# MPF-Optimization-Laboratory/ConicIP.jl

Hardware: NVIDIA B200
Metric: kkt_factor_plus_solves_per_sec (higher is better)
Workload: dtype f64

## Files before the change

conicip.jl_b200/csrc/engine.cu:

```cuda
#include <climits>
#include <stdarg.h>
#include <stdlib.h>
#include <string.h>

#include <math.h>

#include <algorithm>
#include <vector>

#include "engine.h"
#include "nccl_dl.h"

namespace cip {

static thread_local char g_err[1024] = "";
std::atomic<long long> g_launches{0};

int sm_count() {
  static std::atomic<int> cache[64];
  int dev = 0;
  if (cudaGetDevice(&dev) != cudaSuccess || dev < 0 || dev >= 64) return 148;
  int v = cache[dev].load(std::memory_order_relaxed);
  if (v == 0) {
    if (cudaDeviceGetAttribute(&v, cudaDevAttrMultiProcessorCount, dev) != cudaSuccess || v <= 0) v = 148;
// ... 559 lines not shown
    if (cone_type[i] == CIP_CONE_Q) { qlist.push_back(i); maxq = std::max(maxq, cone_dim[i]); }
    else if (cone_type[i] == CIP_CONE_S) {
      const int k = (int)((sqrt(1.0 + 8.0 * cone_dim[i]) - 1.0) / 2.0 + 0.5);
      if (k * (k + 1) / 2 != cone_dim[i]) {
        set_error("S cone %d: dimension %d is not k(k+1)/2", i, cone_dim[i]);
        return -1;
      }
      if (k > sdp_max_order()) {
        set_error("S cone %d: order %d exceeds the supported maximum %d", i, k, sdp_max_order());
        return -2;
      }
      slist.push_back(i);
      h->h_sord.push_back(k);
      h->h_roff.push_back((int)h->r_total);
      h->r_total += (size_t)k * k;
      maxs = std::max(maxs, k);
    }
    else if (cone_type[i] != CIP_CONE_R) {
      set_error("unknown cone type %d", cone_type[i]);
      return -1;
    }
  }
  if (h->h_off[ncones] != m) {
    set_error("cone dimensions sum to %d but A has %d rows", h->h_off[ncones], m);
    return -1;
  }
  CIP_TRY(dev_alloc(h, &h->d_type, ncones));
  CIP_TRY(dev_alloc(h, &h->d_off, ncones + 1));
  CIP_TRY(dev_alloc(h, &h->d_rowcone, m));
  CIP_TRY(dev_alloc(h, &h->d_qlist, qlist.size()));
  CIP_TRY(dev_alloc(h, &h->d_slist, slist.size()));
  CIP_TRY(dev_alloc(h, &h->d_sord, slist.size()));
  CIP_TRY(dev_alloc(h, &h->d_roff, slist.size()));
  h->h_slist = slist;
  if (ncones) CIP_CUDA(cudaMemcpy(h->d_type, h->h_type.data(), sizeof(int) * ncones, cudaMemcpyHostToDevice));
  CIP_CUDA(cudaMemcpy(h->d_off, h->h_off.data(), sizeof(int) * (ncones + 1), cudaMemcpyHostToDevice));
  if (m) CIP_CUDA(cudaMemcpy(h->d_rowcone, rowcone.data(), sizeof(int) * m, cudaMemcpyHostToDevice));
  if (!qlist.empty())
    CIP_CUDA(cudaMemcpy(h->d_qlist, qlist.data(), sizeof(int) * qlist.size(), cudaMemcpyHostToDevice));
  if (!slist.empty()) {
    CIP_CUDA(cudaMemcpy(h->d_slist, slist.data(), sizeof(int) * slist.size(), cudaMemcpyHostToDevice));
    CIP_CUDA(cudaMemcpy(h->d_sord, h->h_sord.data(), sizeof(int) * slist.size(), cudaMemcpyHostToDevice));
    CIP_CUDA(cudaMemcpy(h->d_roff, h->h_roff.data(), sizeof(int) * slist.size(), cudaMemcpyHostToDevice));
  }
  h->cd.m = m; h->cd.ncones = ncones; h->cd.type = h->d_type; h->cd.off = h->d_off;
  h->cd.row_cone = h->d_rowcone; h->cd.qlist = h->d_qlist; h->cd.nq = (int)qlist.size();
  h->cd.slist = h->d_slist; h->cd.ns = (int)slist.size(); h->cd.max_q_dim = maxq; h->cd.max_s_ord = maxs;
  h->cd.sord = h->d_sord; h->cd.roff = h->d_roff;
  h->cd.sws = nullptr; h->cd.sws_stride = sdp_workspace_doubles(maxs);
  if (h->cd.sws_stride > 0) {
    const long long ctas = (long long)slist.size() * std::max(1, sdp_panel_chunks(maxs, n));
    CIP_TRY(dev_alloc(h, &h->d_sws, (size_t)(ctas * h->cd.sws_stride)));
    h->cd.sws = h->d_sws;
  }
  h->cd.nr_rows = 0;
  for (int i = 0; i < ncones; ++i)
    if (cone_type[i] == CIP_CONE_R) h->cd.nr_rows += h->h_off[i + 1] - h->h_off[i];
  for (Scaling* S : {&h->F, &h->Fi}) {
    CIP_TRY(dev_alloc(h, &S->kind, ncones));
    CIP_TRY(dev_alloc(h, &S->a, h->m_pad + 4));
    CIP_TRY(dev_alloc(h, &S->b, h->m_pad + 4));
    CIP_TRY(dev_alloc(h, &S->D, ncones));
  }
  CIP_TRY(dev_alloc(h, &h->F.R, h->r_total));
  CIP_TRY(dev_alloc(h, &h->F.Ri, h->r_total));
  h->Fi.R = h->F.R;
  h->Fi.Ri = h->F.Ri;

  const size_t nn = (size_t)h->n_pad * h->n_pad;
  const size_t mn = (size_t)h->m_pad * h->n_pad;
  if (!(h->rs.on && As)) CIP_TRY(dev_alloc(h, &h->At4, mn));
  {
    double rho = h->opt.aug_rho;
    if (rho < 0) rho = (p > 0) ? 1.0 : 0.0;
    h->aug_rho = (p > 0) ? rho : 0.0;
    h->aug_rows = (h->aug_rho > 0) ? round_up(p, 32) : 0;
  }
  if (!h->rs.on) CIP_TRY(engine_decide_fold(h, slist.empty() && qlist.empty() && h->aug_rows == 0 && m > 0, mn, &h->fold));
  if (!h->rs.on && !h->fold) CIP_TRY(fast_syrk_plan(h, slist.empty() && qlist.empty() && h->aug_rows == 0 && m > 0));
  if (h->fast.on) CIP_TRY(dev_alloc(h, &h->Atil4, fast_syrk_atil_doubles(h)));
  else if (!h->fold && !h->rs.on) CIP_TRY(dev_alloc(h, &h->Atil4, (size_t)(h->m_pad + h->aug_rows) * h->n_pad));
  const bool split = h->rs.sp.on;
  if (!split || (!Qs && h->opt.q_kind == 0)) CIP_TRY(dev_alloc(h, &h->Qq4, nn));
  if (!split) CIP_TRY(dev_alloc(h, &h->H4, nn));
  CIP_TRY(dev_alloc(h, &h->gemm_ws, (size_t)GEMM_WS_DOUBLES));
  if (!split) CIP_TRY(dev_alloc(h, &h->Winv, (size_t)h->n_pad * TILE));
  CIP_TRY(dev_alloc(h, &h->info, 4));
  cudaStream_t s = h->stream;

  if (Qs && split) {
    CIP_TRY(split_classify_csc_Q(h, Qs));
  } else if (Qs) {
    CIP_TRY(upload_csc(h, h->Qq4, h->n_pad, Qs, 0));
  } else if (h->opt.q_kind == 0) {
    if (!Q) { set_error("Q is null"); return -1; }
    if (kernel_readable(Q, h->device)) {
      CIP_TRY(pack_rows_q4(h->Qq4, h->n_pad, Q, ldq, n, n, h->n_pad, h->n_pad, s));
    } else {
      const int chunk = std::max(4, std::min(n, (int)((256u << 20) / ((size_t)n * 8)) / 4 * 4));
      double* stg = nullptr;
      CIP_CUDA(cudaMalloc(&stg, (size_t)n * chunk * 8));
      for (int c0 = 0; c0 < n; c0 += chunk) {
        const int nc = std::min(chunk, n - c0);
        CIP_CUDA(cudaMemcpy2DAsync(stg, (size_t)n * 8, Q + (size_t)c0 * ldq, (size_t)ldq * 8, (size_t)n * 8, nc,
                                   cudaMemcpyDefault, s));
        CIP_TRY(pack_rows_q4(h->Qq4 + (size_t)(c0 / 4) * h->n_pad * 4, h->n_pad, stg, n, n, nc, h->n_pad,
                             round_up(nc, 4), s));
        CIP_CUDA(cudaStreamSynchronize(s));
      }
      cudaFree(stg);
    }
  } else if (h->opt.q_kind == 1) {
    if (!Q) { set_error("Q (diagonal) is null"); return -1; }
    if (split) {
      CIP_TRY(split_diag_Q(h, Q));
    } else {
      double* dq = nullptr;
      CIP_CUDA(cudaMalloc(&dq, sizeof(double) * n));
      CIP_CUDA(cudaMemcpyAsync(dq, Q, sizeof(double) * n, cudaMemcpyDefault, s));
      CIP_TRY(set_diag_vec_q4(h->Qq4, h->n_pad, n, dq, s));
      CIP_CUDA(cudaStreamSynchronize(s));
      cudaFree(dq);
    }
  }
  if (h->Qq4) CIP_TRY(add_diag_q4(h->Qq4, h->n_pad, n, h->n_pad, 1.0, 1, s));

  if (m > 0) {
    if (!A && !As) { set_error("A is null"); return -1; }
    if (As && h->rs.on) {
      CIP_TRY(structure_build_csc(h, As));
    } else if (As) {
      CIP_TRY(upload_csc(h, h->At4, h->n_pad, As, 1));
    } else if (kernel_readable(A, h->device)) {
      CIP_TRY(pack_trans_q4(h->At4, h->n_pad, 0, A, lda, m, h->m_pad, n, s));
    } else {
      const int chunk = std::max(1, std::min(n, (int)((512u << 20) / ((size_t)m * 8))));
      double* stg = nullptr;
      CIP_CUDA(cudaMalloc(&stg, (size_t)m * chunk * 8));
      for (int c0 = 0; c0 < n; c0 += chunk) {
        const int nc = std::min(chunk, n - c0);
        CIP_CUDA(cudaMemcpy2DAsync(stg, (size_t)m * 8, A + (size_t)c0 * lda, (size_t)lda * 8, (size_t)m * 8, nc,
                                   cudaMemcpyDefault, s));
        CIP_TRY(pack_trans_q4(h->At4, h->n_pad, c0, stg, m, m, h->m_pad, nc, s));
        CIP_CUDA(cudaStreamSynchronize(s));
      }
      cudaFree(stg);
    }
    if (h->rs.on && !As) CIP_TRY(structure_build_dense(h));
  }
  if (h->rs.on) {
  } else if (h->fold) {
    CIP_TRY(make_q4_tensor_map(&h->mapAt.map, h->At4, h->n_pad, h->m_pad / 4));
  } else if (h->fast.on) {
    CIP_TRY(make_q4_tensor_map(&h->mapAtil.map, h->Atil4, h->n_pad, (long long)h->fast.K2));
    CIP_TRY(fast_syrk_setup(h));
  } else if (h->m_pad + h->aug_rows > 0) {
    CIP_TRY(make_q4_tensor_map(&h->mapAtil.map, h->Atil4, h->n_pad, (h->m_pad + h->aug_rows) / 4));
  }
  if (!split) CIP_TRY(chol_make_plan(&h->cholH, h->H4, h->n_pad, h->Winv, h->info));

  if (p > 0) {
    if (!G && !Gs) { set_error("G is null"); return -1; }
    const size_t pn = (size_t)h->p_pad * h->n_pad;
    CIP_TRY(dev_alloc(h, &h->G4, pn));
    if (!split) CIP_TRY(dev_alloc(h, &h->Z4, pn));
    CIP_TRY(dev_alloc(h, &h->S4, (size_t)h->p_pad * h->p_pad));
    CIP_TRY(dev_alloc(h, &h->Sbase4, (size_t)h->p_pad * h->p_pad));
    CIP_TRY(dev_alloc(h, &h->WinvS, (size_t)h->p_pad * TILE));
    if (Gs) {
      CIP_TRY(upload_csc(h, h->G4, h->p_pad, Gs, 0));
    } else {
      double* stg = nullptr;
      const double* gsrc = G;
      int gld = ldg;
      if (!kernel_readable(G, h->device)) {
        CIP_CUDA(cudaMalloc(&stg, (size_t)p * n * 8));
        CIP_CUDA(cudaMemcpy2DAsync(stg, (size_t)p * 8, G, (size_t)ldg * 8, (size_t)p * 8, n, cudaMemcpyDefault, s));
        gsrc = stg;
        gld = p;
      }
      CIP_TRY(pack_rows_q4(h->G4, h->p_pad, gsrc, gld, p, n, h->p_pad, h->n_pad, s));
      CIP_CUDA(cudaStreamSynchronize(s));
      if (stg) cudaFree(stg);
    }
    if (h->aug_rows > 0 && !h->rs.on)
      CIP_TRY(transpose_scale_q4(h->Atil4, h->n_pad, h->m_pad, h->G4, h->p_pad, p, n, sqrt(h->aug_rho), s));
    CIP_TRY(add_diag_q4(h->Sbase4, h->p_pad, p, h->p_pad, 1.0, 1, s));
    if (h->opt.reg_eps_G != 0.0) CIP_TRY(add_diag_q4(h->Sbase4, h->p_pad, 0, p, h->opt.reg_eps_G, 1, s));
    if (!split) CIP_TRY(make_q4_tensor_map(&h->mapZ.map, h->Z4, h->p_pad, h->n_pad / 4));
    CIP_TRY(chol_make_plan(&h->cholS, h->S4, h->p_pad, h->WinvS, h->info + 1));
  }
  if (h->rs.on) CIP_TRY(structure_finish(h));

  for (auto& v : h->nv) CIP_TRY(dev_alloc(h, &v, h->n_pad + 4));
  for (auto& v : h->mv) CIP_TRY(dev_alloc(h, &v, h->m_pad + 4));
  for (auto& v : h->pv) CIP_TRY(dev_alloc(h, &v, h->p_pad + 4));
  h->partial_cap = 4 * sm_count() * 8 * 128 + 64 * std::max(n, std::max(p, 1));
  CIP_TRY(dev_alloc(h, &h->partial, h->partial_cap));
  CIP_TRY(dev_alloc(h, &h->scalar, 8));
  CIP_CUDA(cudaStreamSynchronize(s));
  h->st.n = n; h->st.m = m; h->st.p = p; h->st.n_pad = h->n_pad; h->st.m_pad = h->m_pad; h->st.p_pad = h->p_pad;
  return 0;
}

}

namespace cip {
int engine_create_single(cip_handle* out, int n, int m, int p, const double* Q, int ldq, const double* A, int lda,
                         const double* G, int ldg, const cip_csc* Qs, const cip_csc* As, const cip_csc* Gs,
                         int ncones, const int* cone_type, const int* cone_dim, const cip_options* opts) {
  return create_impl(out, n, m, p, Q, ldq, A, lda, G, ldg, Qs, As, Gs, ncones, cone_type, cone_dim, opts,
                     true);
}
}

namespace {
bool wants_multi(const cip_options* opts) {
  return opts && (size_t)opts->struct_size >= offsetof(cip_options, ngpus) + sizeof(int) && opts->ngpus > 1;
}
bool reject_sharded_structure(const cip_options* opts) {
  if (opts && (size_t)opts->struct_size >= offsetof(cip_options, row_structure) + sizeof(int) &&
      opts->row_structure != 0) {
    set_error("row_structure is supported on single-device handles only (ngpus = %d)", opts->ngpus);
    return true;
  }
  return false;
}
}

extern "C" {

int cip_create(cip_handle* out, int n, int m, int p, const double* Q, int ldq, const double* A, int lda,
               const double* G, int ldg, int ncones, const int* cone_type, const int* cone_dim,
               const cip_options* opts) {
  if (wants_multi(opts)) {
    if (!out || n <= 0 || m < 0 || p < 0 || ncones < 0 || (ncones > 0 && (!cone_type || !cone_dim))) {
      set_error("cip_create: bad dimensions n=%d m=%d p=%d ncones=%d", n, m, p, ncones);
      return -1;
    }
    if (reject_sharded_structure(opts)) return -1;
    return multi_create(out, n, m, p, Q, ldq, A, lda, G, ldg, nullptr, nullptr, nullptr, ncones, cone_type,
                        cone_dim, opts);
  }
  return create_impl(out, n, m, p, Q, ldq, A, lda, G, ldg, nullptr, nullptr, nullptr, ncones, cone_type, cone_dim,
                     opts);
}

int cip_create_csc(cip_handle* out, int n, const cip_csc* Q, const cip_csc* A, const cip_csc* G, int ncones,
                   const int* cone_type, const int* cone_dim, const cip_options* opts) {
  if (!A || A->ncols != n || (Q && (Q->nrows != n || Q->ncols != n)) || (G && G->nrows > 0 && G->ncols != n)) {
    set_error("cip_create_csc: inconsistent matrix shapes");
    return -1;
  }
  cip_options o{};
  o.dist_chol = -1;
  o.aug_rho = -1.0;
  if (opts) memcpy(&o, opts, std::min<size_t>(sizeof(o), (size_t)opts->struct_size));
  else o.device = -1;
  o.struct_size = sizeof(o);
  o.q_kind = 2;
  const int p = G ? G->nrows : 0;
  if (wants_multi(&o)) {
    if (!out || n <= 0 || ncones < 0 || (ncones > 0 && (!cone_type || !cone_dim))) {
      set_error("cip_create_csc: bad arguments");
      return -1;
    }
    if (reject_sharded_structure(&o)) return -1;
    return multi_create(out, n, A->nrows, p, nullptr, 0, nullptr, 0, nullptr, 0, Q, A, (p > 0) ? G : nullptr, ncones,
                        cone_type, cone_dim, &o);
  }
  return create_impl(out, n, A->nrows, p, nullptr, 0, nullptr, 0, nullptr, 0, Q, A, (p > 0) ? G : nullptr, ncones,
                     cone_type, cone_dim, &o);
}

int cip_destroy(cip_handle h) {
  if (!h) return 0;
  if (h->multi) return multi_destroy(h);
  cudaSetDevice(h->device);
  if (h->own_stream) cudaStreamSynchronize(h->stream);
  if (h->comm) {
    const NcclApi* api = nccl_api();
    if (api) api->CommDestroy(h->comm);
  }
  void* ptrs[] = {h->At4, h->Atil4, h->Qq4, h->H4, h->Winv, h->G4, h->Z4, h->S4, h->Sbase4, h->WinvS, h->info,
                  h->d_type, h->d_off, h->d_rowcone, h->d_qlist, h->d_slist, h->F.kind, h->F.a, h->F.b, h->F.D,
                  h->Fi.kind, h->Fi.a, h->Fi.b, h->Fi.D, h->partial, h->scalar, h->F.R, h->F.Ri, h->d_sord, h->d_roff, h->gemm_ws};
  for (void* p : ptrs) if (p) cudaFree(p);
  for (void* p : h->owned) cudaFree(p);
  for (auto v : h->nv) if (v) cudaFree(v);
  for (auto v : h->mv) if (v) cudaFree(v);
  for (auto v : h->pv) if (v) cudaFree(v);
  for (auto v : h->nv2) if (v) cudaFree(v);
  for (auto v : h->mv2) if (v) cudaFree(v);
  for (auto v : h->pv2) if (v) cudaFree(v);
  chol_free_plan(&h->cholH);
  chol_free_plan(&h->cholS);
  chol_free_plan(&h->rs.sp.chol);
  if (h->Hp) cudaFree(h->Hp);
  if (h->d_sws) cudaFree(h->d_sws);
  if (h->cs) cudaStreamDestroy(h->cs);
  if (h->s2) cudaStreamDestroy(h->s2);
  for (auto e : h->evc) if (e) cudaEventDestroy(e);
  for (auto e : h->ev) if (e) cudaEventDestroy(e);
  if (h->own_stream) cudaStreamDestroy(h->own_stream);
  cudaGetLastError();
  delete h;
  return 0;
// ... 513 lines not shown
```

conicip.jl_b200/csrc/engine.h:

```cpp
#pragma once
#include <vector>

#include "../../include/conicip_b200.h"
#include "kernels.cuh"

constexpr int NV = 8;
constexpr int MV = 10;
constexpr int PV = 6;

namespace cip {
struct Multi;

struct RowStructure {
  bool on = false;
  int nsing = 0, nempty = 0, nr = 0, nr_pad = 0, nJ = 0, nJ_pad = 0;
  bool compressed = false, base_has_gtg = false, fold = false;
  double *At4r = nullptr, *Atil4r = nullptr, *Hr4 = nullptr;
  double* Base4 = nullptr;
  GemmOperand map{};
  int *rest_row = nullptr, *J = nullptr, *Jinv = nullptr;
  int* row_code = nullptr;
  int *sing_ptr = nullptr, *sing_row = nullptr, *sing_col = nullptr;
  double* sing_val = nullptr;
  ConeDesc cd{};
  int *d_type = nullptr, *d_off = nullptr, *d_rowcone = nullptr, *d_qlist = nullptr, *d_slist = nullptr;
  int* cone_map = nullptr;
  Scaling Fi{};
  double *xr[2] = {}, *yJ[2] = {}, *outr[2] = {}, *outJ[2] = {};

  struct Split {
    bool on = false;
    int nK = 0, nK_pad = 0, from_rest = 0, from_Q = 0, from_G = 0;
    bool g_in_D = false;
    bool factored = false;
    std::vector<int> K;
    std::vector<char> q_couple;
    struct QEntry { int i, j; double v; };
    std::vector<QEntry> qtrip;
    int *dK = nullptr, *Kpos = nullptr, *JK = nullptr;
    double *QK4 = nullptr, *BaseK4 = nullptr, *HK4 = nullptr, *WinvK = nullptr;
    double *qD = nullptr, *hD = nullptr, *kscale = nullptr;
    double *GK4 = nullptr, *ZK4 = nullptr;
    CholPlan chol{};
    GemmOperand mapZK{}, mapG{};
    int* fail = nullptr;
    double* kv[2][3] = {};
  } sp;
};

struct FastSyrk {
  bool on = false;
  int depth = 0;
  int leaf = 0;
  int K2 = 0;
  int nchunk = 0;
  int* colexp = nullptr;
  double* colss = nullptr;
  double* M = nullptr;
  int4* table = nullptr;
};
}

struct cip_engine {
  cip::Multi* multi = nullptr;
  cip::Multi* parent = nullptr;
  int shard_index = 0;
  bool always_sync = false;
  int n = 0, m = 0, p = 0, n_pad = 0, m_pad = 0, p_pad = 0, ncones = 0;
  int device = 0;
  cudaStream_t stream = nullptr, own_stream = nullptr;
  cip_options opt{};
  double *At4 = nullptr, *Atil4 = nullptr, *Qq4 = nullptr, *H4 = nullptr, *Winv = nullptr;
  double *G4 = nullptr, *Z4 = nullptr, *S4 = nullptr, *Sbase4 = nullptr, *WinvS = nullptr;
  cip::GemmOperand mapAtil{}, mapZ{};
  cip::CholPlan cholH{}, cholS{};
  int* info = nullptr;
  std::vector<int> h_type, h_off;
  int *d_type = nullptr, *d_off = nullptr, *d_rowcone = nullptr, *d_qlist = nullptr, *d_slist = nullptr;
  int *d_sord = nullptr, *d_roff = nullptr;
  double* d_sws = nullptr;
  std::vector<int> h_slist, h_sord, h_roff;
  size_t r_total = 0;
  cip::ConeDesc cd{};
  cip::Scaling F{}, Fi{};
  bool have_scaling = false, have_factor = false;
  double* gemm_ws = nullptr;
  bool fold = false;
  cip::GemmOperand mapAt{};
  int aug_rows = 0;
  double aug_rho = 0.0;
  cip::RowStructure rs;
  cip::FastSyrk fast;
  std::vector<void*> owned;
  double* nv[NV] = {};
  double* mv[MV] = {};
  double* pv[PV] = {};
  double* nv2[6] = {};
  double* mv2[6] = {};
  double* pv2[5] = {};
  double* partial = nullptr;
  int partial_cap = 0;
  double* scalar = nullptr;
  void* comm = nullptr;
  int nranks = 1, rank = 0;
  double* Hp = nullptr;
  cudaStream_t cs = nullptr, s2 = nullptr;
  cudaEvent_t evc[16] = {};
  cip_stats_t st{};
  cudaEvent_t ev[8] = {};
  size_t bytes = 0;
  bool need_sync = false;
};


namespace cip {
int engine_allreduce(cip_engine* h, double* buf, size_t count);
int engine_create_single(cip_handle* out, int n, int m, int p, const double* Q, int ldq, const double* A, int lda,
                         const double* G, int ldg, const cip_csc* Qs, const cip_csc* As, const cip_csc* Gs,
                         int ncones, const int* cone_type, const int* cone_dim, const cip_options* opts);
const char* last_error_string();
int engine_decide_fold(cip_engine* h, bool can, size_t mn, bool* fold);
int engine_setup_comm(cip_engine* h);

int fast_syrk_plan(cip_engine* h, bool can);
size_t fast_syrk_atil_doubles(const cip_engine* h);
int fast_syrk_setup(cip_engine* h);
int fast_syrk_drop(cip_engine* h);
int fast_syrk_form(cip_engine* h, const double* cin);

int structure_build_dense(cip_engine* h);
int structure_build_csc(cip_engine* h, const cip_csc* A);
int structure_finish(cip_engine* h);
int structure_form_H(cip_engine* h);
int structure_AT(cip_engine* h, double* out, const double* x, const double* add, int b);
int structure_AT2(cip_engine* h, double* outa, double* outb, const double* xa, const double* xb, const double* adda,
                  const double* addb);
int structure_A(cip_engine* h, double* out, const double* y, int b);
int structure_A2(cip_engine* h, double* outa, double* outb, const double* ya, const double* yb);
int split_classify_csc_Q(cip_engine* h, const cip_csc* Q);
int split_diag_Q(cip_engine* h, const double* q);
int split_build(cip_engine* h);
int split_factor(cip_engine* h);
int split_add_delta(cip_engine* h, double delta);
int split_solve(cip_engine* h, double** nv, double** pv, int b, bool schur);
int split_mul_Q(cip_engine* h, double* y, const double* x);
int split_get_H(cip_engine* h, double* tmp);

int multi_create(cip_handle* out, int n, int m, int p, const double* Q, int ldq, const double* A, int lda,
                 const double* G, int ldg, const cip_csc* Qs, const cip_csc* As, const cip_csc* Gs, int ncones,
                 const int* cone_type, const int* cone_dim, const cip_options* opts);
int multi_destroy(cip_engine* h);
int multi_factor(cip_engine* h, const int* kind, const double* fa, const double* fb, const double* fD,
                 const double* fR, int factor);
int multi_get_scaling(cip_engine* h, int* kind, double* fa, double* fb, double* fD, double* fR);
int multi_nt_scaling(cip_engine* h, const double* v, const double* s, double* lambda_out, int factor);
int multi_solve(cip_engine* h, const double* ry, const double* rw, const double* rv, double* dy, double* dw,
                double* dv);
int multi_solve_multi(cip_engine* h, int nrhs, const double* ry, int ldy, const double* rw, int ldw, const double* rv,
                      int ldv, double* dy, double* dw, double* dv);
int multi_apply(cip_engine* h, int op, const double* x, double* y);
int multi_maxstep(cip_engine* h, const double* x, const double* d, double d_scale, double* alpha_out);
int multi_prod_div(cip_engine* h, const double* x, const double* y, double* o, int divide);
int multi_mul_A(cip_engine* h, int trans, const double* x, double* y);
int multi_mul_GQ(cip_engine* h, int which, int trans, const double* x, double* y);
int multi_ipm_solve(cip_engine* h, const double* c, const double* b, const double* d, const cip_ipm_options* opts,
                    double* y, double* w, double* v, cip_ipm_result* result);
int multi_stats(cip_engine* h, cip_stats_t* out);
int multi_simple(cip_engine* h, int what, double* out, int ldo);
void multi_barrier(cip::Multi* m);
}
```

conicip.jl_b200/csrc/fast_syrk.cu:

```cuda
#include <stdlib.h>

#include <algorithm>
#include <vector>

#include "engine.h"

namespace cip {

namespace {

constexpr int FAST_SYRK_LEAF = 2048;
constexpr int FAST_SYRK_N0 = 12288;

__global__ void __launch_bounds__(256)
winograd_sums_kernel(double* __restrict__ X, int ld, int KQ2, int h, const int* __restrict__ colexp) {
  const int kq = blockIdx.x;
  const int x = blockIdx.y * blockDim.x + threadIdx.x;
  if (x >= ld / 4) return;
  const int p = x / h, i = x - p * h;
  const int ra = 4 * p * h + i, rb = ra + 2 * h;
  auto at = [&](int kqq, int r) { return reinterpret_cast<double2*>(X + ((size_t)kqq * ld + r) * 4); };
  auto ld4 = [&](int kqq, int r, double f, double2& lo, double2& hi) {
    const double2* q = at(kqq, r);
    lo = q[0]; hi = q[1];
    lo.x *= f; lo.y *= f; hi.x *= f; hi.y *= f;
  };
  const double fa1 = ldexp(1.0, -colexp[ra]), fa2 = ldexp(1.0, -colexp[ra + h]);
  const double fb1 = ldexp(1.0, -colexp[rb]), fb2 = ldexp(1.0, -colexp[rb + h]);
  double2 a11l, a11h, a12l, a12h, a21l, a21h, a22l, a22h, b11l, b11h, b12l, b12h, b21l, b21h, b22l, b22h;
  ld4(kq, rb, fb1, a11l, a11h);
  ld4(kq + KQ2, rb, fb1, a12l, a12h);
  ld4(kq, rb + h, fb2, a21l, a21h);
  ld4(kq + KQ2, rb + h, fb2, a22l, a22h);
  ld4(kq, ra, fa1, b11l, b11h);
  ld4(kq + KQ2, ra, fa1, b12l, b12h);
  ld4(kq, ra + h, fa2, b21l, b21h);
  ld4(kq + KQ2, ra + h, fa2, b22l, b22h);
  auto add = [](double2 u, double2 v) { return make_double2(u.x + v.x, u.y + v.y); };
  auto sub = [](double2 u, double2 v) { return make_double2(u.x - v.x, u.y - v.y); };
  const double2 s1l = add(a21l, a22l), s1h = add(a21h, a22h);
  const double2 s2l = sub(s1l, a11l), s2h = sub(s1h, a11h);
  const double2 s3l = sub(a11l, a21l), s3h = sub(a11h, a21h);
  const double2 s4l = sub(a12l, s2l), s4h = sub(a12h, s2h);
  const double2 t1l = sub(b21l, b11l), t1h = sub(b21h, b11h);
  const double2 t2l = sub(b22l, t1l), t2h = sub(b22h, t1h);
  const double2 t3l = sub(b22l, b21l), t3h = sub(b22h, b21h);
  const double2 t4l = sub(t2l, b12l), t4h = sub(t2h, b12h);
  const int ks = 2 * KQ2 + kq, kt = 3 * KQ2 + kq;
  auto st4 = [&](int kqq, int r, double2 lo, double2 hi) { double2* q = at(kqq, r); q[0] = lo; q[1] = hi; };
  st4(ks, ra, s1l, s1h);
  st4(ks, ra + h, s2l, s2h);
  st4(ks, ra + 2 * h, s3l, s3h);
  st4(ks, ra + 3 * h, s4l, s4h);
  st4(kt, ra, t1l, t1h);
  st4(kt, ra + h, t2l, t2h);
  st4(kt, ra + 2 * h, t3l, t3h);
  st4(kt, ra + 3 * h, t4l, t4h);
}

__global__ void __launch_bounds__(256)
winograd_combine_kernel(const double* __restrict__ M, const double* __restrict__ Cin, double* __restrict__ H, int ld,
                        int h, const int* __restrict__ colexp) {
  const int nt = h / TILE, G = nt * nt;
  const int L = blockIdx.x, p = blockIdx.y;
  const int ti = L % nt, tj = L / nt;
  const int ra = 4 * p * h, rb = ra + 2 * h;
  const size_t slab = (size_t)TILE * TILE;
  const double* Mp = M + ((size_t)p * 7 * G + L) * slab;
  for (int e = threadIdx.x * 2; e < TILE * TILE; e += 512) {
    const int quad = e / (TILE * 4), lr = (e % (TILE * 4)) >> 2, c = e & 3;
    const int i = ti * TILE + lr, j = tj * TILE + quad * 4 + c;
    double2 P[7];
#pragma unroll
    for (int q = 0; q < 7; ++q) P[q] = *reinterpret_cast<const double2*>(Mp + (size_t)q * G * slab + e);
    const int eb1 = colexp[rb + i], eb2 = colexp[rb + h + i];
    const int ea1[2] = {colexp[ra + j], colexp[ra + j + 1]};
    const int ea2[2] = {colexp[ra + h + j], colexp[ra + h + j + 1]};
    double o[4][2];
#pragma unroll
    for (int k = 0; k < 2; ++k) {
      const double p1 = k ? P[0].y : P[0].x, p2 = k ? P[1].y : P[1].x, p3 = k ? P[2].y : P[2].x;
      const double p4 = k ? P[3].y : P[3].x, p5 = k ? P[4].y : P[4].x, p6 = k ? P[5].y : P[5].x;
      const double p7 = k ? P[6].y : P[6].x;
      const double u2 = ldexp(p1, -(eb1 + ea1[k])) + p6;
      const double u3 = u2 + p7, u4 = u2 + p5;
      o[0][k] = p1 + p2;
      o[1][k] = ldexp(u4 + ldexp(p3, -ea2[k]), eb1 + ea2[k]);
      o[2][k] = ldexp(u3 - ldexp(p4, -eb2), eb2 + ea1[k]);
      o[3][k] = ldexp(u3 + p5, eb2 + ea2[k]);
    }
#pragma unroll
    for (int b = 0; b < 4; ++b) {
      const size_t idx = q4_index(rb + (b >> 1) * h + i, ra + (b & 1) * h + j, ld);
      double2 v = make_double2(o[b][0], o[b][1]);
      if (Cin) {
        const double2 q = *reinterpret_cast<const double2*>(Cin + idx);
        v.x += q.x;
        v.y += q.y;
      }
      *reinterpret_cast<double2*>(H + idx) = v;
    }
  }
}

int env_int(const char* name, int dflt) {
  const char* e = getenv(name);
  return (e && *e) ? atoi(e) : dflt;
}

template <typename T>
int falloc(cip_engine* h, T** p, size_t count) {
  *p = nullptr;
  if (count == 0) count = 1;
  CIP_CUDA(cudaMalloc(reinterpret_cast<void**>(p), count * sizeof(T)));
  CIP_CUDA(cudaMemsetAsync(*p, 0, count * sizeof(T), h->stream));
  h->bytes += count * sizeof(T);
  h->owned.push_back(*p);
  return 0;
}

size_t m_doubles(int n_pad) { return (size_t)7 * n_pad / 4 * n_pad / 4; }

}

int fast_syrk_plan(cip_engine* h, bool can) {
  FastSyrk& f = h->fast;
  f = FastSyrk{};
  const int mode = env_int("CIP_FAST_SYRK", 2);
  if (!can || mode == 0 || h->m_pad == 0) return 0;
  int leaf = std::max(256, env_int("CIP_FAST_SYRK_LEAF", FAST_SYRK_LEAF));
  if (mode == 1) leaf = std::min(leaf, h->n_pad / 2);
  int W = h->n_pad, depth = 0;
  while (W % 512 == 0 && W / 2 >= leaf) { W /= 2; ++depth; }
  if (depth == 0 || (mode != 1 && h->n_pad < FAST_SYRK_N0)) return 0;
  const int K2 = round_up(h->m_pad, 64) / 2;
  const size_t nn = (size_t)h->n_pad * h->n_pad;
  const size_t atil = (size_t)4 * K2 * h->n_pad;
  const size_t colss = (size_t)scale_panel_norms_chunks(h->m_pad) * h->n_pad;
  if (mode != 1) {
    size_t free_b = 0, total_b = 0;
    CIP_CUDA(cudaMemGetInfo(&free_b, &total_b));
    const size_t need = (atil + m_doubles(h->n_pad) + colss + 3 * nn + (size_t)GEMM_WS_DOUBLES) * 8 + (size_t(1) << 30);
    if (free_b < need) return 0;
  }
  f.on = true;
  f.depth = depth;
  f.leaf = W;
  f.K2 = K2;
  f.nchunk = scale_panel_norms_chunks(h->m_pad);
  return 0;
}

size_t fast_syrk_atil_doubles(const cip_engine* h) { return (size_t)4 * h->fast.K2 * h->n_pad; }

int fast_syrk_setup(cip_engine* h) {
  FastSyrk& f = h->fast;
  if (!f.on) return 0;
  CIP_TRY(falloc(h, &f.colexp, h->n_pad));
  CIP_TRY(falloc(h, &f.colss, (size_t)f.nchunk * h->n_pad));
  CIP_TRY(falloc(h, &f.M, m_doubles(h->n_pad)));
  const int KQ2 = f.K2 / 4, PQ0 = 2 * KQ2;
  std::vector<int4> t;
  for (int l = 0; l < (1 << f.depth); ++l) {
    const int r0 = l * f.leaf;
    t.push_back(make_int4(r0, 0, r0, 0));
    t.push_back(make_int4(r0, r0, 0, 0));
  }
  for (int d = 0; d < f.depth; ++d) {
    const int w = h->n_pad >> (d + 1), hh = w / 2;
    for (int p = 0; p < (1 << d); ++p) {
      const int ra = 2 * p * w, rb = ra + w;
      const int4 ops[7] = {
          make_int4(rb, 0, ra, 0),
          make_int4(rb, KQ2, ra, KQ2),
          make_int4(ra + 3 * hh, PQ0, ra + hh, KQ2),
          make_int4(rb + hh, KQ2, ra + 3 * hh, PQ0 + KQ2),
          make_int4(ra, PQ0, ra, PQ0 + KQ2),
          make_int4(ra + hh, PQ0, ra + hh, PQ0 + KQ2),
          make_int4(ra + 2 * hh, PQ0, ra + 2 * hh, PQ0 + KQ2)};
      for (const int4& o : ops) {
        t.push_back(o);
        t.push_back(make_int4(0, 0, 0, 0));
      }
    }
  }
  CIP_TRY(falloc(h, &f.table, t.size()));
  CIP_CUDA(cudaMemcpyAsync(f.table, t.data(), t.size() * sizeof(int4), cudaMemcpyHostToDevice, h->stream));
  CIP_CUDA(cudaStreamSynchronize(h->stream));
  return 0;
}

int fast_syrk_drop(cip_engine* h) {
  FastSyrk& f = h->fast;
  if (!f.on) return 0;
  CIP_CUDA(cudaStreamSynchronize(h->stream));
  for (void* p : {(void*)f.colexp, (void*)f.colss, (void*)f.M, (void*)f.table}) {
    h->owned.erase(std::find(h->owned.begin(), h->owned.end(), p));
    CIP_CUDA(cudaFree(p));
  }
  CIP_CUDA(cudaFree(h->Atil4));
  h->bytes -= fast_syrk_atil_doubles(h) * 8;
  const size_t mn = (size_t)h->m_pad * h->n_pad;
  CIP_CUDA(cudaMalloc(reinterpret_cast<void**>(&h->Atil4), mn * 8));
  CIP_CUDA(cudaMemsetAsync(h->Atil4, 0, mn * 8, h->stream));
  h->bytes += mn * 8;
  CIP_TRY(make_q4_tensor_map(&h->mapAtil.map, h->Atil4, h->n_pad, h->m_pad / 4));
  f = FastSyrk{};
  return 0;
}

int fast_syrk_form(cip_engine* h, const double* cin) {
  const FastSyrk& f = h->fast;
  cudaStream_t s = h->stream;
  const int KQ2 = f.K2 / 4, L = 1 << f.depth;
  for (int d = 0; d < f.depth; ++d) {
    const int pairs = 1 << d, hh = h->n_pad >> (d + 2), nt = hh / TILE;
    winograd_sums_kernel<<<dim3(KQ2, (h->n_pad / 4 + 255) / 256), 256, 0, s>>>(h->Atil4, h->n_pad, KQ2, hh, f.colexp);
    CIP_CHECK_LAUNCH();
    GemmArgs g{};
    g.lower = 0; g.ntm = g.ntn = nt; g.sym = 0;
    g.nk = f.K2 / 32;
    g.Ctm = f.M; g.ldc = h->n_pad; g.alpha = 1.0;
    g.ws = h->gemm_ws; g.ws_doubles = GEMM_WS_DOUBLES;
    g.group = f.table + 2 * (L + 7 * (pairs - 1));
    g.group_tiles = nt * nt;
    g.tile_count = 7 * pairs * nt * nt;
    CIP_TRY(launch_gemm_nt(h->mapAtil, h->mapAtil, g, s));
    winograd_combine_kernel<<<dim3(nt * nt, pairs), 256, 0, s>>>(f.M, cin, h->H4, h->n_pad, hh, f.colexp);
    CIP_CHECK_LAUNCH();
  }
  const int T = f.leaf / TILE;
  GemmArgs a{};
  a.lower = 1; a.ntm = a.ntn = T; a.sym = 1;
  a.nk = h->m_pad / 32;
  a.Cin = cin; a.Cout = h->H4; a.ldc = h->n_pad; a.alpha = 1.0;
  a.ws = h->gemm_ws; a.ws_doubles = GEMM_WS_DOUBLES;
  a.group = f.table;
  a.group_tiles = T * (T + 1) / 2;
  a.tile_count = L * a.group_tiles;
  CIP_TRY(launch_gemm_nt(h->mapAtil, h->mapAtil, a, s));
  return 0;
}

}
```

Baseline: 0.5459.

## Add second recursive Winograd level to fast SYRK off-diagonal products

Each off-diagonal Strassen-Winograd product in the fast SYRK path is now itself computed with another Winograd step when the half-block is large enough. Seven smaller GEMMs replace each large one, and new sums and combine kernels plus an extra M2 scratch buffer and extra Atil rows hold the intermediate operands. The aim is fewer FP64 multiply flops when forming H. In exchange it adds more kernel launches, more memory traffic and scratch memory, and some loss of numerical accuracy. Exponent scaling is folded into the combine steps to keep accuracy under control.

```diff
diff --git a/conicip.jl_b200/csrc/engine.cu b/conicip.jl_b200/csrc/engine.cu
--- a/conicip.jl_b200/csrc/engine.cu
+++ b/conicip.jl_b200/csrc/engine.cu
@@ -735,7 +735,7 @@
   } else if (h->fold) {
     CIP_TRY(make_q4_tensor_map(&h->mapAt.map, h->At4, h->n_pad, h->m_pad / 4));
   } else if (h->fast.on) {
-    CIP_TRY(make_q4_tensor_map(&h->mapAtil.map, h->Atil4, h->n_pad, (long long)h->fast.K2));
+    CIP_TRY(make_q4_tensor_map(&h->mapAtil.map, h->Atil4, h->n_pad, (long long)(fast_syrk_atil_doubles(h) / h->n_pad / 4)));
     CIP_TRY(fast_syrk_setup(h));
   } else if (h->m_pad + h->aug_rows > 0) {
     CIP_TRY(make_q4_tensor_map(&h->mapAtil.map, h->Atil4, h->n_pad, (h->m_pad + h->aug_rows) / 4));
diff --git a/conicip.jl_b200/csrc/engine.h b/conicip.jl_b200/csrc/engine.h
--- a/conicip.jl_b200/csrc/engine.h
+++ b/conicip.jl_b200/csrc/engine.h
@@ -53,10 +53,12 @@
   int depth = 0;
   int leaf = 0;
   int K2 = 0;
+  unsigned two = 0;
   int nchunk = 0;
   int* colexp = nullptr;
   double* colss = nullptr;
   double* M = nullptr;
+  double* M2 = nullptr;
   int4* table = nullptr;
 };
 }
diff --git a/conicip.jl_b200/csrc/fast_syrk.cu b/conicip.jl_b200/csrc/fast_syrk.cu
--- a/conicip.jl_b200/csrc/fast_syrk.cu
+++ b/conicip.jl_b200/csrc/fast_syrk.cu
@@ -11,31 +11,41 @@
 
 constexpr int FAST_SYRK_LEAF = 2048;
 constexpr int FAST_SYRK_N0 = 12288;
-
-__global__ void __launch_bounds__(256)
-winograd_sums_kernel(double* __restrict__ X, int ld, int KQ2, int h, const int* __restrict__ colexp) {
+constexpr int FAST_SYRK_L2_MIN = 1024;
+
+struct SumsArgs {
+  int h, kqh, pstride, count;
+  int a_row, a_kq, b_row, b_kq, s_row, s_kq, t_row, t_kq;
+  int scale_a, scale_b;
+};
+
+__device__ __forceinline__ void winograd_sums(double* __restrict__ X, int ld, const SumsArgs& s,
+                                              const int* __restrict__ colexp) {
   const int kq = blockIdx.x;
   const int x = blockIdx.y * blockDim.x + threadIdx.x;
-  if (x >= ld / 4) return;
-  const int p = x / h, i = x - p * h;
-  const int ra = 4 * p * h + i, rb = ra + 2 * h;
+  if (x >= s.count) return;
+  const int h = s.h, KQ2 = s.kqh;
+  const int p = x / h, i = x - p * h, base = p * s.pstride;
+  const int xa = base + s.a_row + i, xb = base + s.b_row + i;
+  const int ka = s.a_kq + kq, kb = s.b_kq + kq;
   auto at = [&](int kqq, int r) { return reinterpret_cast<double2*>(X + ((size_t)kqq * ld + r) * 4); };
   auto ld4 = [&](int kqq, int r, double f, double2& lo, double2& hi) {
     const double2* q = at(kqq, r);
     lo = q[0]; hi = q[1];
     lo.x *= f; lo.y *= f; hi.x *= f; hi.y *= f;
   };
-  const double fa1 = ldexp(1.0, -colexp[ra]), fa2 = ldexp(1.0, -colexp[ra + h]);
-  const double fb1 = ldexp(1.0, -colexp[rb]), fb2 = ldexp(1.0, -colexp[rb + h]);
+  auto fac = [&](int on, int r) { return on ? ldexp(1.0, -colexp[r]) : 1.0; };
+  const double fa1 = fac(s.scale_a, xa), fa2 = fac(s.scale_a, xa + h);
+  const double fb1 = fac(s.scale_b, xb), fb2 = fac(s.scale_b, xb + h);
   double2 a11l, a11h, a12l, a12h, a21l, a21h, a22l, a22h, b11l, b11h, b12l, b12h, b21l, b21h, b22l, b22h;
-  ld4(kq, rb, fb1, a11l, a11h);
-  ld4(kq + KQ2, rb, fb1, a12l, a12h);
-  ld4(kq, rb + h, fb2, a21l, a21h);
-  ld4(kq + KQ2, rb + h, fb2, a22l, a22h);
-  ld4(kq, ra, fa1, b11l, b11h);
-  ld4(kq + KQ2, ra, fa1, b12l, b12h);
-  ld4(kq, ra + h, fa2, b21l, b21h);
-  ld4(kq + KQ2, ra + h, fa2, b22l, b22h);
+  ld4(ka, xa, fa1, a11l, a11h);
+  ld4(ka + KQ2, xa, fa1, a12l, a12h);
+  ld4(ka, xa + h, fa2, a21l, a21h);
+  ld4(ka + KQ2, xa + h, fa2, a22l, a22h);
+  ld4(kb, xb, fb1, b11l, b11h);
+  ld4(kb + KQ2, xb, fb1, b12l, b12h);
+  ld4(kb, xb + h, fb2, b21l, b21h);
+  ld4(kb + KQ2, xb + h, fb2, b22l, b22h);
   auto add = [](double2 u, double2 v) { return make_double2(u.x + v.x, u.y + v.y); };
   auto sub = [](double2 u, double2 v) { return make_double2(u.x - v.x, u.y - v.y); };
   const double2 s1l = add(a21l, a22l), s1h = add(a21h, a22h);
@@ -46,21 +56,71 @@
   const double2 t2l = sub(b22l, t1l), t2h = sub(b22h, t1h);
   const double2 t3l = sub(b22l, b21l), t3h = sub(b22h, b21h);
   const double2 t4l = sub(t2l, b12l), t4h = sub(t2h, b12h);
-  const int ks = 2 * KQ2 + kq, kt = 3 * KQ2 + kq;
+  const int ks = s.s_kq + kq, kt = s.t_kq + kq, rs = base + s.s_row + i, rt = base + s.t_row + i;
   auto st4 = [&](int kqq, int r, double2 lo, double2 hi) { double2* q = at(kqq, r); q[0] = lo; q[1] = hi; };
-  st4(ks, ra, s1l, s1h);
-  st4(ks, ra + h, s2l, s2h);
-  st4(ks, ra + 2 * h, s3l, s3h);
-  st4(ks, ra + 3 * h, s4l, s4h);
-  st4(kt, ra, t1l, t1h);
-  st4(kt, ra + h, t2l, t2h);
-  st4(kt, ra + 2 * h, t3l, t3h);
-  st4(kt, ra + 3 * h, t4l, t4h);
+  st4(ks, rs, s1l, s1h);
+  st4(ks, rs + h, s2l, s2h);
+  st4(ks, rs + 2 * h, s3l, s3h);
+  st4(ks, rs + 3 * h, s4l, s4h);
+  st4(kt, rt, t1l, t1h);
+  st4(kt, rt + h, t2l, t2h);
+  st4(kt, rt + 2 * h, t3l, t3h);
+  st4(kt, rt + 3 * h, t4l, t4h);
+}
+
+__global__ void __launch_bounds__(256)
+winograd_sums_kernel(double* __restrict__ X, int ld, const SumsArgs s, const int* __restrict__ colexp) {
+  winograd_sums(X, ld, s, colexp);
+}
+__global__ void __launch_bounds__(256)
+winograd_sums2_kernel(double* __restrict__ X, int ld, const SumsArgs s, const int* __restrict__ colexp) {
+  winograd_sums(X, ld, s, colexp);
+}
+
+__global__ void __launch_bounds__(256)
+winograd_combine2_kernel(const double* __restrict__ M2, double* __restrict__ M, int h2, int q, int pstride,
+                         int x_row, int y_row, int raw_x, int raw_y, const int* __restrict__ colexp) {
+  const int nt2 = h2 / TILE, G2 = nt2 * nt2, nt = 2 * nt2, G = nt * nt;
+  const int L2 = blockIdx.x, p = blockIdx.y;
+  const int ti = L2 % nt2, tj = L2 / nt2;
+  const int xr = p * pstride + x_row, yr = p * pstride + y_row;
+  const size_t slab = (size_t)TILE * TILE;
+  const double* Mp = M2 + ((size_t)p * 7 * G2 + L2) * slab;
+  double* Mq = M + (size_t)(p * 7 + q) * G * slab;
+  for (int e = threadIdx.x * 2; e < TILE * TILE; e += 512) {
+    const int quad = e / (TILE * 4), lr = (e % (TILE * 4)) >> 2, c = e & 3;
+    const int i = ti * TILE + lr, j = tj * TILE + quad * 4 + c;
+    double2 P[7];
+#pragma unroll
+    for (int r = 0; r < 7; ++r) P[r] = *reinterpret_cast<const double2*>(Mp + (size_t)r * G2 * slab + e);
+    const int ex1 = raw_x ? colexp[xr + i] : 0, ex2 = raw_x ? colexp[xr + h2 + i] : 0;
+    const int ey1[2] = {raw_y ? colexp[yr + j] : 0, raw_y ? colexp[yr + j + 1] : 0};
+    const int ey2[2] = {raw_y ? colexp[yr + h2 + j] : 0, raw_y ? colexp[yr + h2 + j + 1] : 0};
+    double o[4][2];
+#pragma unroll
+    for (int k = 0; k < 2; ++k) {
+      const double p1 = k ? P[0].y : P[0].x, p2 = k ? P[1].y : P[1].x, p3 = k ? P[2].y : P[2].x;
+      const double p4 = k ? P[3].y : P[3].x, p5 = k ? P[4].y : P[4].x, p6 = k ? P[5].y : P[5].x;
+      const double p7 = k ? P[6].y : P[6].x;
+      const double s1 = ldexp(p1, -(ex1 + ey1[k])), s2 = ldexp(p2, -(ex1 + ey1[k]));
+      const double u2 = s1 + p6;
+      const double u3 = u2 + p7, u4 = u2 + p5;
+      o[0][k] = s1 + s2;
+      o[1][k] = u4 + ldexp(p3, -ey2[k]);
+      o[2][k] = u3 - ldexp(p4, -ex2);
+      o[3][k] = u3 + p5;
+    }
+#pragma unroll
+    for (int b = 0; b < 4; ++b) {
+      const int L = (ti + (b >> 1) * nt2) + (tj + (b & 1) * nt2) * nt;
+      *reinterpret_cast<double2*>(Mq + (size_t)L * slab + e) = make_double2(o[b][0], o[b][1]);
+    }
+  }
 }
 
 __global__ void __launch_bounds__(256)
 winograd_combine_kernel(const double* __restrict__ M, const double* __restrict__ Cin, double* __restrict__ H, int ld,
-                        int h, const int* __restrict__ colexp) {
+                        int h, int scaled, const int* __restrict__ colexp) {
   const int nt = h / TILE, G = nt * nt;
   const int L = blockIdx.x, p = blockIdx.y;
   const int ti = L % nt, tj = L / nt;
@@ -82,11 +142,11 @@
       const double p1 = k ? P[0].y : P[0].x, p2 = k ? P[1].y : P[1].x, p3 = k ? P[2].y : P[2].x;
       const double p4 = k ? P[3].y : P[3].x, p5 = k ? P[4].y : P[4].x, p6 = k ? P[5].y : P[5].x;
       const double p7 = k ? P[6].y : P[6].x;
-      const double u2 = ldexp(p1, -(eb1 + ea1[k])) + p6;
+      const double u2 = (scaled ? p1 : ldexp(p1, -(eb1 + ea1[k]))) + p6;
       const double u3 = u2 + p7, u4 = u2 + p5;
-      o[0][k] = p1 + p2;
-      o[1][k] = ldexp(u4 + ldexp(p3, -ea2[k]), eb1 + ea2[k]);
-      o[2][k] = ldexp(u3 - ldexp(p4, -eb2), eb2 + ea1[k]);
+      o[0][k] = scaled ? ldexp(p1 + p2, eb1 + ea1[k]) : p1 + p2;
+      o[1][k] = ldexp(u4 + (scaled ? p3 : ldexp(p3, -ea2[k])), eb1 + ea2[k]);
+      o[2][k] = ldexp(u3 - (scaled ? p4 : ldexp(p4, -eb2)), eb2 + ea1[k]);
       o[3][k] = ldexp(u3 + p5, eb2 + ea2[k]);
     }
 #pragma unroll
@@ -120,6 +180,36 @@
 }
 
 size_t m_doubles(int n_pad) { return (size_t)7 * n_pad / 4 * n_pad / 4; }
+
+size_t m2_doubles(int n_pad, unsigned two) {
+  if (!two) return 0;
+  int d = 0;
+  while (!(two >> d & 1u)) ++d;
+  const size_t h2 = (size_t)n_pad >> (d + 3);
+  return (size_t)7 * ((size_t)1 << d) * h2 * h2;
+}
+
+size_t atil_rows(const FastSyrk& f) { return (size_t)4 * f.K2 + (f.two ? f.K2 / 2 : 0); }
+
+void winograd_ops(int4 ops[7], int xr, int xk, int yr, int yk, int hh, int kqh, int sr, int sk, int tr, int tk) {
+  ops[0] = make_int4(xr, xk, yr, yk);
+  ops[1] = make_int4(xr, xk + kqh, yr, yk + kqh);
+  ops[2] = make_int4(sr + 3 * hh, sk, yr + hh, yk + kqh);
+  ops[3] = make_int4(xr + hh, xk + kqh, tr + 3 * hh, tk);
+  ops[4] = make_int4(sr, sk, tr, tk);
+  ops[5] = make_int4(sr + hh, sk, tr + hh, tk);
+  ops[6] = make_int4(sr + 2 * hh, sk, tr + 2 * hh, tk);
+}
+
+void level1_ops(int4 ops[7], int p, int hh, int KQ2) {
+  const int ra = 4 * p * hh, rb = ra + 2 * hh;
+  winograd_ops(ops, rb, 0, ra, 0, hh, KQ2, ra, 2 * KQ2, ra, 3 * KQ2);
+}
+
+void level2_ops(int4 ops[7], int4 o, int p, int hh, int KQ2) {
+  const int ra = 4 * p * hh;
+  winograd_ops(ops, o.x, o.y, o.z, o.w, hh / 2, KQ2 / 2, ra, 4 * KQ2, ra + 2 * hh, 4 * KQ2);
+}
 
 }
 
@@ -133,25 +223,33 @@
   int W = h->n_pad, depth = 0;
   while (W % 512 == 0 && W / 2 >= leaf) { W /= 2; ++depth; }
   if (depth == 0 || (mode != 1 && h->n_pad < FAST_SYRK_N0)) return 0;
-  const int K2 = round_up(h->m_pad, 64) / 2;
+  const int levels = env_int("CIP_FAST_SYRK_LEVELS", 0);
+  unsigned two = 0;
+  for (int d = 0; d < depth && levels != 1; ++d) {
+    const int h2 = h->n_pad >> (d + 3);
+    if (h2 % TILE == 0 && (h2 >= FAST_SYRK_L2_MIN || levels == 2)) two |= 1u << d;
+  }
   const size_t nn = (size_t)h->n_pad * h->n_pad;
-  const size_t atil = (size_t)4 * K2 * h->n_pad;
   const size_t colss = (size_t)scale_panel_norms_chunks(h->m_pad) * h->n_pad;
-  if (mode != 1) {
+  for (;; two = 0) {
+    f.two = two;
+    f.K2 = round_up(h->m_pad, two ? 128 : 64) / 2;
+    if (mode == 1) break;
     size_t free_b = 0, total_b = 0;
     CIP_CUDA(cudaMemGetInfo(&free_b, &total_b));
-    const size_t need = (atil + m_doubles(h->n_pad) + colss + 3 * nn + (size_t)GEMM_WS_DOUBLES) * 8 + (size_t(1) << 30);
-    if (free_b < need) return 0;
+    const size_t need = (atil_rows(f) * h->n_pad + m_doubles(h->n_pad) + m2_doubles(h->n_pad, two) + colss + 3 * nn +
+                         (size_t)GEMM_WS_DOUBLES) * 8 + (size_t(1) << 30);
+    if (free_b >= need) break;
+    if (!two) { f = FastSyrk{}; return 0; }
   }
   f.on = true;
   f.depth = depth;
   f.leaf = W;
-  f.K2 = K2;
   f.nchunk = scale_panel_norms_chunks(h->m_pad);
   return 0;
 }
 
-size_t fast_syrk_atil_doubles(const cip_engine* h) { return (size_t)4 * h->fast.K2 * h->n_pad; }
+size_t fast_syrk_atil_doubles(const cip_engine* h) { return atil_rows(h->fast) * h->n_pad; }
 
 int fast_syrk_setup(cip_engine* h) {
   FastSyrk& f = h->fast;
@@ -159,31 +257,38 @@
   CIP_TRY(falloc(h, &f.colexp, h->n_pad));
   CIP_TRY(falloc(h, &f.colss, (size_t)f.nchunk * h->n_pad));
   CIP_TRY(falloc(h, &f.M, m_doubles(h->n_pad)));
-  const int KQ2 = f.K2 / 4, PQ0 = 2 * KQ2;
+  if (f.two) CIP_TRY(falloc(h, &f.M2, m2_doubles(h->n_pad, f.two)));
+  const int KQ2 = f.K2 / 4;
   std::vector<int4> t;
   for (int l = 0; l < (1 << f.depth); ++l) {
     const int r0 = l * f.leaf;
     t.push_back(make_int4(r0, 0, r0, 0));
     t.push_back(make_int4(r0, r0, 0, 0));
   }
+  int4 ops[7], sub[7];
   for (int d = 0; d < f.depth; ++d) {
-    const int w = h->n_pad >> (d + 1), hh = w / 2;
+    const int hh = h->n_pad >> (d + 2);
     for (int p = 0; p < (1 << d); ++p) {
-      const int ra = 2 * p * w, rb = ra + w;
-      const int4 ops[7] = {
-          make_int4(rb, 0, ra, 0),
-          make_int4(rb, KQ2, ra, KQ2),
-          make_int4(ra + 3 * hh, PQ0, ra + hh, KQ2),
-          make_int4(rb + hh, KQ2, ra + 3 * hh, PQ0 + KQ2),
-          make_int4(ra, PQ0, ra, PQ0 + KQ2),
-          make_int4(ra + hh, PQ0, ra + hh, PQ0 + KQ2),
-          make_int4(ra + 2 * hh, PQ0, ra + 2 * hh, PQ0 + KQ2)};
+      level1_ops(ops, p, hh, KQ2);
       for (const int4& o : ops) {
         t.push_back(o);
         t.push_back(make_int4(0, 0, 0, 0));
       }
     }
   }
+  for (int d = 0; d < f.depth; ++d) {
+    if (!(f.two >> d & 1u)) continue;
+    const int hh = h->n_pad >> (d + 2);
+    for (int q = 0; q < 7; ++q)
+      for (int p = 0; p < (1 << d); ++p) {
+        level1_ops(ops, p, hh, KQ2);
+        level2_ops(sub, ops[q], p, hh, KQ2);
+        for (const int4& o : sub) {
+          t.push_back(o);
+          t.push_back(make_int4(0, 0, 0, 0));
+        }
+      }
+  }
   CIP_TRY(falloc(h, &f.table, t.size()));
   CIP_CUDA(cudaMemcpyAsync(f.table, t.data(), t.size() * sizeof(int4), cudaMemcpyHostToDevice, h->stream));
   CIP_CUDA(cudaStreamSynchronize(h->stream));
@@ -194,7 +299,8 @@
   FastSyrk& f = h->fast;
   if (!f.on) return 0;
   CIP_CUDA(cudaStreamSynchronize(h->stream));
-  for (void* p : {(void*)f.colexp, (void*)f.colss, (void*)f.M, (void*)f.table}) {
+  for (void* p : {(void*)f.colexp, (void*)f.colss, (void*)f.M, (void*)f.M2, (void*)f.table}) {
+    if (!p) continue;
     h->owned.erase(std::find(h->owned.begin(), h->owned.end(), p));
     CIP_CUDA(cudaFree(p));
   }
@@ -213,9 +319,12 @@
   const FastSyrk& f = h->fast;
   cudaStream_t s = h->stream;
   const int KQ2 = f.K2 / 4, L = 1 << f.depth;
+  int sub_entry = L + 7 * (L - 1);
   for (int d = 0; d < f.depth; ++d) {
     const int pairs = 1 << d, hh = h->n_pad >> (d + 2), nt = hh / TILE;
-    winograd_sums_kernel<<<dim3(KQ2, (h->n_pad / 4 + 255) / 256), 256, 0, s>>>(h->Atil4, h->n_pad, KQ2, hh, f.colexp);
+    const bool two = f.two >> d & 1u;
+    SumsArgs sa{hh, KQ2, 4 * hh, pairs * hh, 2 * hh, 0, 0, 0, 0, 2 * KQ2, 0, 3 * KQ2, 1, 1};
+    winograd_sums_kernel<<<dim3(KQ2, (sa.count + 255) / 256), 256, 0, s>>>(h->Atil4, h->n_pad, sa, f.colexp);
     CIP_CHECK_LAUNCH();
     GemmArgs g{};
     g.lower = 0; g.ntm = g.ntn = nt; g.sym = 0;
@@ -225,8 +334,33 @@
     g.group = f.table + 2 * (L + 7 * (pairs - 1));
     g.group_tiles = nt * nt;
     g.tile_count = 7 * pairs * nt * nt;
-    CIP_TRY(launch_gemm_nt(h->mapAtil, h->mapAtil, g, s));
-    winograd_combine_kernel<<<dim3(nt * nt, pairs), 256, 0, s>>>(f.M, cin, h->H4, h->n_pad, hh, f.colexp);
+    if (!two) {
+      CIP_TRY(launch_gemm_nt(h->mapAtil, h->mapAtil, g, s));
+    } else {
+      const int h2 = hh / 2, nt2 = h2 / TILE;
+      int4 ops[7];
+      level1_ops(ops, 0, hh, KQ2);
+      for (int q = 0; q < 7; ++q) {
+        const int4 o = ops[q];
+        const int raw_x = o.y < 2 * KQ2, raw_y = o.w < 2 * KQ2;
+        SumsArgs s2{h2, KQ2 / 2, 4 * hh, pairs * h2, o.x, o.y, o.z, o.w, 0, 4 * KQ2, 2 * hh, 4 * KQ2, raw_x, raw_y};
+        winograd_sums2_kernel<<<dim3(KQ2 / 2, (s2.count + 255) / 256), 256, 0, s>>>(h->Atil4, h->n_pad, s2, f.colexp);
+        CIP_CHECK_LAUNCH();
+        GemmArgs g2 = g;
+        g2.ntm = g2.ntn = nt2;
+        g2.nk = f.K2 / 64;
+        g2.Ctm = f.M2;
+        g2.group = f.table + 2 * sub_entry;
+        g2.group_tiles = nt2 * nt2;
+        g2.tile_count = 7 * pairs * nt2 * nt2;
+        sub_entry += 7 * pairs;
+        CIP_TRY(launch_gemm_nt(h->mapAtil, h->mapAtil, g2, s));
+        winograd_combine2_kernel<<<dim3(nt2 * nt2, pairs), 256, 0, s>>>(f.M2, f.M, h2, q, 4 * hh, o.x, o.z, raw_x,
+                                                                        raw_y, f.colexp);
+        CIP_CHECK_LAUNCH();
+      }
+    }
+    winograd_combine_kernel<<<dim3(nt * nt, pairs), 256, 0, s>>>(f.M, cin, h->H4, h->n_pad, hh, two, f.colexp);
     CIP_CHECK_LAUNCH();
   }
   const int T = f.leaf / TILE;
```

Measured after the change: 0.5823 (median of 6 runs). +6.7%, better.
